# Kyo-suke-S/Depth_image_captioning_pub

Measured on AMD Instinct MI355X. Metric: images/sec (train, depth-soft, 224x224, seq-len 20), higher is better.
Workload: dtype f32; 1 GPU; depth-soft train step, synthetic RGB-D 224x224, batch 64/GPU, seq-len 20, V=10000, ResNet-152 (random init, batch-stat BN) + depth CNN + soft-attention LSTM; global_batch=64, batch_per_gpu=64, seq_len=20, vocab=10000, parallelism=dp1, resnet_conv_mode=f16x2, cross_step_resnet_overlap=True, resnet_forwards_in_flight=3, annotation_cells=49, ranks=1, collective=none (single rank)

## Files before the change

### depth_image_captioning_pub_amd/csrc/api.hip

```cpp
#include "dic.h"
#include "conv.h"
#include "nn_kernels.h"

#include <cstdio>

using namespace dic;

namespace dic { void resnet_fuse_bn_operand(int mask); void resnet_fuse_bn_halo(int on); void resnet_fuse_res_bn(int on); void depth_encoder_l1_sparse(int on); void bn_finalize_two_level_rows(int rows); void resnet_debug_fused_tail_bn(int on); void conv1_depth_debug_blocks(int n);
                void depth_encoder_f16x2(int on); }
#ifdef DIC_EXPERIMENTS
namespace dic { void decoder_debug_persistent(int on); void decoder_persist_debug_buffer(unsigned long long* p); void decoder_persist_debug_placement(int p);
                void resnet_debug_skip_bn_apply(int on); }
#endif

extern "C" {

int dic_version(void) { return DIC_ABI_VERSION; }
size_t dic_struct_bytes(int which) {
  switch (which) {
    case 0: return sizeof(dic_conv_bn_layer);
    case 1: return sizeof(dic_decoder_weights);
    case 2: return sizeof(dic_decoder_grads);
    case 3: return sizeof(dic_depth_encoder_weights);
    case 4: return sizeof(dic_depth_encoder_grads);
// ... 24 lines not shown
}

int dic_conv2d_fwd(const float* x, int B, int H, int W, int C, int in_nchw, const float* w_ohwi, const float* bias,
                   int CO, int KH, int KW, int stride, int pad, float* y_nhwc, float* bn_partial, int* mtiles_out,
                   int force_tile, float* tail_ws, void* stream) {
  ConvDesc d{B, H, W, C, CO, KH, KW, stride, pad, in_nchw};
  return conv_fwd(x, d, w_ohwi, bias, y_nhwc, bn_partial, mtiles_out, (hipStream_t)stream, force_tile, tail_ws);
}

int dic_debug_force_staged_gemm(int on) {
  if (gemm_bf3_force_tile(on) == 0) return 0;
  if (on >= 100 && on <= 104) { dic::resnet_fuse_bn_operand(on == 104 ? -1 : on - 100); return 0; }
  if (on == 98 || on == 99) { dic::resnet_fuse_res_bn(on - 98); return 0; }
  if (on == 108 || on == 109) { dic::resnet_fuse_bn_halo(on - 108); return 0; }
  if (on == 182 || on == 183) { dic::bn_finalize_two_level_rows(on == 182 ? 512 : 1024); return 0; }
  if (on == 180 || on == 181) { dic::depth_encoder_l1_sparse(on - 180); return 0; }
  if (on == 116 || on == 117) { dic::depth_encoder_f16x2(on - 116); return 0; }
#ifdef DIC_EXPERIMENTS
  if (on == 140 || on == 141) { dic::decoder_debug_persistent(on - 140); return 0; }
  if (on == 142 || on == 143) { dic::decoder_persist_debug_placement(on - 142); return 0; }
  if (on >= 130 && on <= 134) { dic::conv1_depth_debug_blocks(256 * (on - 130)); return 0; }
  if (on >= 150 && on <= 153) { dic::resnet_debug_fused_tail_bn(on - 150); return 0; }
  if (on >= 124 && on <= 127) { dic::resnet_debug_skip_bn_apply(on == 125 ? 3 : on == 126 ? 2 : on == 127 ? 1 : 0); return 0; }
  if (on >= 0 && on <= 13) { gemm_force_v1(on); return 0; }
#endif
  DIC_REQUIRE(false, "debug switch: unknown code %d", on);
  return 0;
}
#ifdef DIC_EXPERIMENTS
int dic_debug_decoder_stamps(unsigned long long* dev_buf) { dic::decoder_persist_debug_buffer(dev_buf); return 0; }
#endif
int dic_debug_conv1_wgrad(const float* x, int B, int H, int W, const float* dy, float* dw, float* dbias, float* ws, float* cs_ws,
                          void* stream) {
  ConvDesc d{B, H, W, 1, 128, 7, 7, 3, 0, 0};
  return conv1_depth_wgrad(x, d, dy, dw, dbias, ws, cs_ws, (hipStream_t)stream);
}
int dic_debug_conv1_fwd(const float* x, int B, int H, int W, const float* w, const float* bias, float* y, float* partial,
                        void* stream) {
  ConvDesc d{B, H, W, 1, 128, 7, 7, 3, 0, 0};
  int rows = 0;
  return conv1_depth_fwd(x, d, w, bias, y, partial, &rows, (hipStream_t)stream);
}
// ... 355 lines not shown
```

### depth_image_captioning_pub_amd/csrc/decoder.h

```cpp
#pragma once
#include "dic.h"
#include "gemm.h"
#include <vector>

namespace dic {

constexpr int kL = DIC_L, kD = DIC_D, kA = DIC_A, kE = DIC_E, kH = DIC_H;
constexpr int kG = 4 * kH;
constexpr int kXK = kE + kD + kH;
constexpr int kNCH = kD / 256;
constexpr int kLCH = 4;
constexpr int kLc = 49;
constexpr int kS_LSTM = 18;
constexpr int kS_DX = 4;

struct SetupBufs {
  float *F, *P, *mean, *Wcat, *WcatT, *bcat, *WhT, *WbT, *gemm_ws;
  size_t gemm_ws_floats;
};

struct DecoderWs : SetupBufs {
  float *WzT, *Xall, *Hall, *Call, *Gact, *Qall, *ctx, *gate, *Hdrop;
  float* slab_g;
  float *dHd, *dG, *slab_dx, *dctx, *dgpre, *dq, *dalp, *pbeta, *dqp, *dwf_acc, *dbf_acc, *dPacc, *carry_dc;
// ... 21 lines not shown
    constexpr int L_ = kL;              \
    STMT                                \
  } else {                              \
    constexpr int L_ = kLc;             \
    STMT                                \
  }

struct StepPlan { int T = 0, N = 0; std::vector<int> bs, off; };
int make_plan(const int* dec_len, int B, StepPlan* pl);

int launch_transpose(const float* in, float* out, int R, int Cc, hipStream_t st);
int gemm(int M, int N, int K, GemmOperand A, GemmOperand B, GemmEpilogue ep, hipStream_t st, int splitk = 1, float* ws = nullptr,
         int tile = 0, int raw_partials = 0);
int gemm_slabs(int M, int N, int K, GemmOperand A, GemmOperand B, float* slabs, int splitk, hipStream_t st);

struct InitState { float *h0, *c0; long long ld; bool WcatT; };
int decoder_setup(const dic_decoder_weights* w, const float* feat_rgb, const float* feat_depth, int B, int cells,
                  const SetupBufs& s, const InitState& o, hipStream_t st);

struct LstmCell {
  const float *slab, *bcat, *drop; float *Hall, *Call, *Gact, *Hdrop;
  int nslab, nb, packed_off;
};
int launch_lstm_fwd(const LstmCell& c, int t, int T, hipStream_t st);

struct FusedLstm : LstmCell { int nb_cur; };

struct AttnStepArgs {
  const float *F, *P, *Hall, *WhT, *b_h, *w_full, *b_full, *WbT, *b_beta;
  int t, T, mode; const float* gumbel_u; int B; float temp;
// ... 131 lines not shown
```

### depth_image_captioning_pub_amd/csrc/decoder_bwd.hip

```cpp
#include "decoder.h"
#include <algorithm>

namespace dic {

__global__ void __launch_bounds__(256) colsum_kernel(const float* __restrict__ X, long long ld, int M, int N,
                                                      float* __restrict__ out, int rs) {
  const int n = blockIdx.x * 256 + threadIdx.x;
  if (n >= N) return;
  float s = 0.f;
#pragma unroll 8
  for (int m = blockIdx.y; m < M; m += rs) s += X[(long long)m * ld + n];
  out[(long long)blockIdx.y * N + n] = s;
}

__global__ void __launch_bounds__(256) colsum_batch_kernel(const ColsumBatch b, int stage) {
  const ColsumJob job = b.j[blockIdx.z];
  const int n = blockIdx.x * 256 + threadIdx.x, y = blockIdx.y;
  if (n >= job.N) return;
  if (stage == 1) {
    if (y >= job.rs) return;
    float s = 0.f;
#pragma unroll 8
    for (int m = y; m < job.M; m += job.rs) s += job.X[(long long)m * job.ld + n];
    (job.rs > 1 ? job.part : job.out)[(long long)y * job.N + n] = s;
// ... 20 lines not shown
  if (maxrs > 1) hipLaunchKernelGGL(colsum_batch_kernel, dim3(ceil_div(maxn, 256), 1, njobs), dim3(256), 0, st, b, 2);
  DIC_LAUNCH_CHECK();
  return DIC_OK;
}

static int colsum(const float* X, long long ld, int M, int N, float* out, float* ws, hipStream_t st) {
  const int rs = std::min(64, std::max(1, M / 8));
  if (rs > 1) {
    hipLaunchKernelGGL(colsum_kernel, dim3(ceil_div(N, 256), rs), dim3(256), 0, st, X, ld, M, N, ws, rs);
    hipLaunchKernelGGL(colsum_kernel, dim3(ceil_div(N, 256), 1), dim3(256), 0, st, ws, (long long)N, rs, N, out, 1);
  } else {
    hipLaunchKernelGGL(colsum_kernel, dim3(ceil_div(N, 256), 1), dim3(256), 0, st, X, ld, M, N, out, 1);
  }
  DIC_LAUNCH_CHECK();
  return DIC_OK;
}

__global__ void __launch_bounds__(kH) lstm_bwd_kernel(const LstmBwdArgs la) { lstm_bwd_body(blockIdx.x, threadIdx.x, true, la); }

template <int L>
__global__ void __launch_bounds__(512, 4) attn_bwd_a_kernel(
    const float* __restrict__ F, const float* __restrict__ slab_dx, int nslab, int nb, int B, int t, int T,
    const float* __restrict__ ctx_all, const float* __restrict__ gate_all, const float* __restrict__ W_beta,
    const long long* __restrict__ cap, int cap_stride, int V, float* __restrict__ dctx_all,
    float* __restrict__ dgpre_all, float* __restrict__ dalp, float* __restrict__ pbeta, float* __restrict__ dembed) {
  __shared__ __align__(16) float dctx_s[256];
  __shared__ float dgp_s[256];
  __shared__ float pb_s[4][kH];
  __shared__ float da_s[256];
  const int chunk = blockIdx.x, b = blockIdx.y;
// ... 395 lines not shown
  DIC_REQUIRE(w != nullptr && workspace != nullptr, "decoder: null weights/workspace");
  DIC_REQUIRE(V > 0 && B > 0, "decoder: bad sizes");
  DIC_REQUIRE(g && dlogits_packed && alphas_in && captions, "decoder_bwd: null pointer");
  DIC_REQUIRE(mode == 0 || mode == 1, "decoder_bwd: only soft (0) and gumbel-softmax (1) attention are differentiable");
  StepPlan pl;
  DIC_TRY(make_plan(dec_lengths, B, &pl));
  const int T = pl.T, N = pl.N;
  DIC_REQUIRE(T <= 64, "decoder_bwd: at most 64 decode steps supported (got %d)", T);
  bool ov = false;
  DecoderWs ws = decoder_carve(workspace, workspace_bytes, B, T, V, N, &ov);
  DIC_REQUIRE(!ov, "decoder_bwd: workspace too small");
  const size_t BT = (size_t)B * T;

  int* d_len = ws.dlen;
  DIC_CHECK_HIP(hipMemcpyAsync(d_len, dec_lengths, sizeof(int) * B, hipMemcpyHostToDevice, st));
  DIC_CHECK_HIP(hipMemsetAsync(ws.dG, 0, (size_t)((char*)(ws.dq + BT * kA) - (char*)ws.dG), st));
  DIC_CHECK_HIP(hipMemsetAsync(g->embed, 0, sizeof(float) * (size_t)V * kE, st));
  float* cs = ws.colsum_ws;
  if (cells != kL) {
    alphas = ws.alpha_c;
    if (dalphas_in) {
      const long long n = (long long)B * T * kLc;
      hipLaunchKernelGGL(fold_dalphas_kernel, dim3((unsigned)((n + 255) / 256)), dim3(256), 0, st, dalphas_in, ws.dalpha_c, n);
      DIC_LAUNCH_CHECK();
      dalphas = ws.dalpha_c;
    }
  }

  DIC_TRY(gemm(N, kH, V, op_rowk(dlogits_packed, V), op_colk(w->out_w, kH), ep_store(ws.dHd, kH), st, 8, ws.gemm_ws));
  DIC_TRY(gemm(V, kH, N, op_colk(dlogits_packed, V), op_colk(ws.Hdrop, kH), ep_store(g->out_w, kH), st));
  DIC_TRY(colsum(dlogits_packed, V, N, V, g->out_b, cs, st));

  const float inv_temp = (mode == 1) ? 1.0f / temp : 1.0f;
  const bool fuse_b = (nlch == 1);
  auto lstm_args = [&](int t) {
    LstmBwdArgs a{};
    a.T = T; a.B = B; a.nlch = nlch; a.dHd = ws.dHd; a.drop = drop_mult; a.slab_dx = ws.slab_dx; a.nslab_dx = kS_DX;
    a.dqp = ws.dqp; a.pbeta = ws.pbeta; a.W_h = w->dec_att_w; a.Gact = ws.Gact; a.Call = ws.Call; a.carry_dc = ws.carry_dc;
    a.dG = ws.dG; a.dq_all = ws.dq; a.dinit = ws.dinit;
    if (t < 0) { a.t = -1; a.nb_next = pl.bs[0]; a.have_next = 1; a.final_pass = 1; a.packed_off = 0; a.nb_slab = pl.bs[0]; }
    else {
      a.t = t; a.have_next = (t + 1 < T); a.nb_next = a.have_next ? pl.bs[t + 1] : 0; a.final_pass = 0;
      a.packed_off = pl.off[t]; a.nb_slab = a.nb_next;
    }
    return a;
  };
// ... 119 lines not shown
```

### depth_image_captioning_pub_amd/csrc/gemm.h

```cpp
#pragma once
#include "common.h"

namespace dic {

__host__ __device__ __forceinline__ long long plane_offset(long long r, long long k, long long kblocks, int paired) {
  if (!paired) return r * kblocks * 32 + k;
  return (((r >> 1) * kblocks + (k >> 5)) << 6) + ((r & 1) << 5) + (k & 31);
}

enum : int { OPK_ROWK = 0, OPK_COLK = 1, OPK_IM2COL = 2, OPK_GATHER = 3, OPK_IM2COL_COLK = 4, OPK_GATHER_COLK = 5 };
enum : int { ACT_NONE = 0, ACT_RELU = 1, ACT_SIGMOID = 2, ACT_GELU = 3 };

struct ConvGeom {
  int H, W, C;
  int OH, OW;
  int KH, KW, stride, pad;
  int nchw;
};

struct GemmOperand {
  const float* p;
  long long ld;
  int kind;
  int vec;
// ... 16 lines not shown
};

struct GemmParams {
  int M, N, K;
  GemmOperand A, B;
  GemmEpilogue ep;
  int mtiles, ntiles;
  int splitk;
  int ktiles_per_split;
  float* ws;
  int tail_first_block, tail_first_tile, tail_split;
  float* tail_ws;
  int ablate;
  int raw_partials;
  int tail128_first, tail128_ntiles;
};

size_t gemm_splitk_ws_bytes(int M, int N, int splitk);
constexpr size_t kGemmTailWsBytes = (size_t)256 * 64 * 64 * sizeof(float);
int gemm_pick_tile(int M, int N);
int gemm_launch(GemmParams p, hipStream_t st, int force_tile = 0);
constexpr int kGemmGroupMax = 6;
int gemm_launch_group_colk(GemmParams* ps, int n, hipStream_t st);
GemmOperand op_rowk(const float* p, long long ld);
GemmOperand op_colk(const float* p, long long ld);
GemmOperand op_im2col(const float* x, const ConvGeom& g);
GemmOperand op_gather(const float* x, const ConvGeom& g);
GemmOperand op_im2col_colk(const float* x, const ConvGeom& g);
GemmOperand op_gather_colk(const float* x, const ConvGeom& g);
void gemm_force_v1(int on);
int gemm_bf3_set_persist_grid(int workgroups);
int gemm_bf3_force_tile(int code);
int gemm_launch_tail_fixup(const GemmParams& p, int tail_tiles, hipStream_t st);

struct BnFuseArgs {
// ... 25 lines not shown
```

### depth_image_captioning_pub_amd/csrc/gemm.hip

```cpp
#include "gemm.h"
#include "gemm_epilogue.h"
#include <algorithm>
#include <map>
#include <vector>

namespace dic {

constexpr int BK = 32;

template <int KIND>
struct KFast { static constexpr bool v = (KIND == OPK_ROWK || KIND == OPK_IM2COL || KIND == OPK_GATHER); };

template <int KIND, int BR>
struct Loader {
  static constexpr bool KFAST = KFast<KIND>::v;
  static constexpr int LD = KFAST ? BR + 1 : BR + 4;
  static constexpr int NV = BR / 32;
  static constexpr int I4 = BR / 4;
  static constexpr int KSTEP = 256 / I4;

  const float* p;
  long long ld;
  int R, K, vec;
  ConvGeom g;
// ... 530 lines not shown
    const float sc = bn.gamma[c] * invstd;
    bn.scale[c] = sc;
    bn.shift[c] = bn.beta[c] - (float)mean * sc;
    bn.mean[c] = (float)mean;
    bn.invstd[c] = invstd;
    const bool finite = fabs(a) <= 1.7e308 && fabs(b) <= 1.7e308;
    if (!finite) f16x2_raise(bn.status, 8u);
    if (bn.running_mean && finite) {
      const double unb = bn.count > 1.0 ? var * bn.count / (bn.count - 1.0) : var;
      bn.running_mean[c] = fmaf(1.f - bn.momentum, bn.running_mean[c], __fmul_rn(bn.momentum, (float)mean));
      bn.running_var[c] = fmaf(1.f - bn.momentum, bn.running_var[c], __fmul_rn(bn.momentum, (float)unb));
    }
  }
}

template <int BM, int BN, int AK, int BKIND, int ABL = 0>
__device__ __forceinline__ void gemm_tile_body(const GemmParams& p, const int bid, const int nblk) {
  using LA = Loader<AK, BM>;
  using LB = Loader<BKIND, BN>;
  constexpr int LDA = LA::LD, LDB = LB::LD;
  constexpr int WM = BM / 2, WN = BN / 2, TM = WM / 32, TN = WN / 32;
  __shared__ __align__(16) float As[2][BK * LDA];
  __shared__ __align__(16) float Bs[2][BK * LDB];

  const int tid = threadIdx.x, lane = tid & 63, wave = tid >> 6;
  const int wm = wave >> 1, wn = wave & 1;
  const int lb = xcd_remap(bid, nblk);
  const int tiles = p.mtiles * p.ntiles;
  const int z = lb / tiles, t = lb - z * tiles;
  const int tm = t / p.ntiles, tn = t - tm * p.ntiles;

  LA la;
// ... 16 lines not shown
  }

  const int nk = (p.K + BK - 1) / BK;
  const int kt0 = z * p.ktiles_per_split;
  const int kt1 = min(nk, kt0 + p.ktiles_per_split);

  f32x16 acc[TM][TN];
#pragma unroll
  for (int i = 0; i < TM; ++i)
#pragma unroll
    for (int j = 0; j < TN; ++j)
#pragma unroll
      for (int r = 0; r < 16; ++r) acc[i][j][r] = 0.f;

  float4 ra[LA::NV], rb[LB::NV];
  const int nkt = kt1 - kt0;
  if (nkt > 0) {
    la.load(kt0 * BK, ra);
    lbld.load(kt0 * BK, rb);
    la.store(As[0], ra);
    lbld.store(Bs[0], rb);
  }
  if (nkt > 1) {
    la.load((kt0 + 1) * BK, ra);
    lbld.load((kt0 + 1) * BK, rb);
  }
  __syncthreads();

  const int arow = wm * WM + (lane & 31);
  const int brow = wn * WN + (lane & 31);
  const int khalf = lane >> 5;
  for (int it = 0; it < nkt; ++it) {
    const int cur = it & 1;
    if (ABL == 0 || ABL == 3) {
    if (it + 1 < nkt) {
      la.store(As[cur ^ 1], ra);
      lbld.store(Bs[cur ^ 1], rb);
    }
    if (it + 2 < nkt && ABL == 0) {
      la.load((kt0 + it + 2) * BK, ra);
      lbld.load((kt0 + it + 2) * BK, rb);
    }
    }
    const float* Ac = As[cur] + khalf * LDA + arow;
    const float* Bc = Bs[cur] + khalf * LDB + brow;
    float af[TM][BK / 2], bf[TN][BK / 2];
#pragma unroll
    for (int kk = 0; kk < BK / 2; ++kk) {
#pragma unroll
      for (int i = 0; i < TM; ++i) af[i][kk] = (ABL == 2) ? (float)(it + kk + i) : Ac[kk * 2 * LDA + i * 32];
#pragma unroll
      for (int j = 0; j < TN; ++j) bf[j][kk] = (ABL == 2) ? (float)(it - kk + j) : Bc[kk * 2 * LDB + j * 32];
    }
    __builtin_amdgcn_sched_barrier(0);
#pragma unroll
    for (int kk = 0; kk < BK / 2; ++kk)
#pragma unroll
      for (int i = 0; i < TM; ++i)
#pragma unroll
        for (int j = 0; j < TN; ++j)
          acc[i][j] = __builtin_amdgcn_mfma_f32_32x32x2f32(af[i][kk], bf[j][kk], acc[i][j], 0, 0, 0);
    __syncthreads();
  }

  gemm_epilogue<BM, BN>(p, acc, tm, tn, z, As[0]);
}

template <int BM, int BN, int AK, int BKIND, int ABL = 0>
__global__ void __launch_bounds__(256) gemm_kernel(const GemmParams p) {
  gemm_tile_body<BM, BN, AK, BKIND, ABL>(p, blockIdx.x, gridDim.x);
}

struct GemmGroup {
  int n;
  int first[kGemmGroupMax + 1];
  GemmParams p[kGemmGroupMax];
};
static_assert(sizeof(GemmGroup) <= 4096, "GemmGroup travels as a kernel argument");
template <int BM, int BN, int AK, int BKIND>
__global__ void __launch_bounds__(256) gemm_group_kernel(const GemmGroup g) {
  int i = 0;
#pragma unroll
  for (int j = 1; j < kGemmGroupMax; ++j)
    if (j < g.n && (int)blockIdx.x >= g.first[j]) i = j;
  gemm_tile_body<BM, BN, AK, BKIND>(g.p[i], (int)blockIdx.x - g.first[i], g.first[i + 1] - g.first[i]);
}

__device__ __forceinline__ void splitk_reduce_body(const GemmParams& p, const int bid, const int nblk) {
  const long long total = (long long)p.M * p.N;
  const float alpha = ep_alpha(p.ep);
  for (long long e = (long long)bid * 256 + threadIdx.x; e < total; e += (long long)nblk * 256) {
    float s = 0.f;
    for (int z = 0; z < p.splitk; ++z) s += p.ws[(long long)z * total + e];
    const int m = (int)(e / p.N), n = (int)(e - (long long)m * p.N);
    finalize_store(p.ep, m, n, s, alpha);
  }
}
__global__ void __launch_bounds__(256) splitk_reduce_kernel(const GemmParams p) { splitk_reduce_body(p, blockIdx.x, gridDim.x); }
__global__ void __launch_bounds__(256) splitk_reduce_group_kernel(const GemmGroup g) {
  int i = 0;
#pragma unroll
  for (int j = 1; j < kGemmGroupMax; ++j)
    if (j < g.n && (int)blockIdx.x >= g.first[j]) i = j;
  splitk_reduce_body(g.p[i], (int)blockIdx.x - g.first[i], g.first[i + 1] - g.first[i]);
}

struct ProfRec { hipEvent_t e0, e1; double flops; int key; double bytes; };
static bool g_prof_on = false;
static bool g_force_v1 = false;
static int g_dma_stages = 2;
static bool g_tail_split_on = true;
// ... 96 lines not shown
  GemmEpilogue e{};
  e.C = C; e.ldc = ldc; e.bias = bias; e.act = act; e.alpha = 1.0f;
  return e;
}

size_t gemm_splitk_ws_bytes(int M, int N, int splitk) {
  return splitk > 1 ? (size_t)splitk * M * N * sizeof(float) : 0;
}

int gemm_pick_tile(int M, int N) {
  const long long t128 = (long long)ceil_div(M, 128) * ceil_div(N, 128);
  if (N >= 128 && M >= 128 && t128 >= 4096) return 128;
  return 64;
}

template <int BM, int BN>
static int launch_tile(const GemmParams& p, hipStream_t st) {
  const dim3 grid(p.mtiles * p.ntiles * p.splitk), block(256);
  const int a = p.A.kind, b = p.B.kind;
#define DIC_GEMM_CASE(AK_, BK_)                                                     \
  if (a == AK_ && b == BK_) {                                                       \
    hipLaunchKernelGGL((gemm_kernel<BM, BN, AK_, BK_>), grid, block, 0, st, p);     \
    return DIC_OK;                                                                  \
  }
  if (a == OPK_ROWK && b == OPK_ROWK && p.ablate > 0) {
    if (p.ablate == 1) hipLaunchKernelGGL((gemm_kernel<BM, BN, OPK_ROWK, OPK_ROWK, 1>), grid, block, 0, st, p);
    else if (p.ablate == 2) hipLaunchKernelGGL((gemm_kernel<BM, BN, OPK_ROWK, OPK_ROWK, 2>), grid, block, 0, st, p);
    else hipLaunchKernelGGL((gemm_kernel<BM, BN, OPK_ROWK, OPK_ROWK, 3>), grid, block, 0, st, p);
    return DIC_OK;
  }
// ... 42 lines not shown
  if (p.A.kind == OPK_IM2COL) DIC_REQUIRE(p.A.g.C % 32 == 0, "im2col loader needs C %% 32 == 0 (C=%d)", p.A.g.C);
  const bool taps_ok = p.A.kind != OPK_IM2COL || p.A.g.KH * p.A.g.KW <= 32;
  if (p.B.kind == OPK_IM2COL_COLK) DIC_REQUIRE(p.B.g.C % 4 == 0, "im2col_colk loader needs C %% 4 == 0");
  const int tile = force_tile ? force_tile : gemm_pick_tile(p.M, p.N);
  p.mtiles = ceil_div(p.M, tile);
  p.ntiles = ceil_div(p.N, tile);
  const int nk = ceil_div(p.K, BK);
  if (p.splitk < 1) p.splitk = 1;
  if (p.splitk > nk) p.splitk = nk;
  p.ktiles_per_split = ceil_div(nk, p.splitk);
  p.splitk = ceil_div(nk, p.ktiles_per_split);
  if (p.splitk > 1) {
    DIC_REQUIRE(p.ws != nullptr, "gemm: split-K needs a workspace");
    DIC_REQUIRE(p.ep.stats == nullptr, "gemm: BN statistics epilogue cannot be combined with split-K");
  }
  if (p.ep.alpha == 0.0f) p.ep.alpha = 1.0f;
  const bool dma_ok = (p.B.kind == OPK_ROWK && p.B.vec && (p.K % 4 == 0) && p.ablate == 0 && !g_force_v1 && taps_ok &&
                       (p.A.kind == OPK_IM2COL || (p.A.kind == OPK_ROWK && p.A.vec)));
  int total_blocks = p.mtiles * p.ntiles * p.splitk;
  p.tail_first_block = total_blocks; p.tail_first_tile = 0; p.tail_split = 1;
  int tail_tiles = 0;
  if (dma_ok && tile == 64 && p.splitk == 1 && p.tail_ws != nullptr && g_tail_split_on) {
    const int T = p.mtiles * p.ntiles, r = T % 256;
    int s = r > 0 ? 256 / r : 0;
    s = std::min(s, std::min(nk / 2, kTailMaxSplit));
    if (r > 0 && r <= 128 && s >= 2 && T < 7 * 256) {
      tail_tiles = r;
      p.tail_first_tile = T - r;
      p.tail_first_block = T - r;
      p.tail_split = s;
// ... 12 lines not shown
  int rc = DIC_OK;
  if (dma_ok) {
    const dim3 grid(total_blocks), block(256);
    if (tile == 128) {
      if (p.A.kind == OPK_IM2COL) hipLaunchKernelGGL((gemm_dma_kernel<128, 128, OPK_IM2COL, 2>), grid, block, 0, st, p);
      else hipLaunchKernelGGL((gemm_dma_kernel<128, 128, OPK_ROWK, 2>), grid, block, 0, st, p);
    } else if (p.raw_partials && p.A.kind == OPK_ROWK && p.mtiles == 1 && p.ktiles_per_split <= 8) {
      hipLaunchKernelGGL((gemm_dma_kernel<64, 64, OPK_ROWK, 4>), grid, block, 0, st, p);
    } else if (g_dma_stages == 2) {
      if (p.A.kind == OPK_IM2COL) hipLaunchKernelGGL((gemm_dma_kernel<64, 64, OPK_IM2COL, 2>), grid, block, 0, st, p);
      else hipLaunchKernelGGL((gemm_dma_kernel<64, 64, OPK_ROWK, 2>), grid, block, 0, st, p);
    } else {
      if (p.A.kind == OPK_IM2COL) hipLaunchKernelGGL((gemm_dma_kernel<64, 64, OPK_IM2COL, 3>), grid, block, 0, st, p);
      else hipLaunchKernelGGL((gemm_dma_kernel<64, 64, OPK_ROWK, 3>), grid, block, 0, st, p);
    }
  } else {
    rc = (tile == 128) ? launch_tile<128, 128>(p, st) : launch_tile<64, 64>(p, st);
  }
  if (rc != 0) return rc;
  DIC_LAUNCH_CHECK();
  if (tail_tiles > 0 && !g_tail_skip_fix) {
    const dim3 g(tail_tiles), b(1024);
  if (p.tail_split <= 2) hipLaunchKernelGGL(tail_fixup_kernel<2>, g, b, 0, st, p);
  else if (p.tail_split <= 4) hipLaunchKernelGGL(tail_fixup_kernel<4>, g, b, 0, st, p);
  else if (p.tail_split <= 8) hipLaunchKernelGGL(tail_fixup_kernel<8>, g, b, 0, st, p);
  else hipLaunchKernelGGL(tail_fixup_kernel<16>, g, b, 0, st, p);
    DIC_LAUNCH_CHECK();
  }
  if (g_prof_on) {
    (void)hipEventRecord(rec.e1, st);
// ... 64 lines not shown
```

### depth_image_captioning_pub_amd/csrc/nic_train.hip

```cpp
#include "nic.h"
#include <algorithm>

namespace dic {

struct NicTape {
  float *G0, *C0, *H0, *H0p, *G1, *C1, *H1p, *Hdrop;
};

__global__ void __launch_bounds__(kNicThreads) nic_lstm2_seq_fwd(const float* __restrict__ Gx0, const float* __restrict__ Whh0p,
                                                                  const float* __restrict__ Wih1p, const float* __restrict__ Whh1p,
                                                                  const float* __restrict__ b1, const int* __restrict__ dlen,
                                                                  const int* __restrict__ off, const float* __restrict__ drop,
                                                                  int B, int T, NicTape tp) {
  __shared__ __align__(16) float h0_s[kNicR][kH];
  __shared__ __align__(16) float h1_s[kNicR][kH];
  __shared__ __align__(16) float g_s[kNicR][kG];
  const int tid = threadIdx.x, b0 = blockIdx.x * kNicR;
  const int rc = tid >> 7, u = tid & (kH - 1), bc = b0 + rc;
  const __amdgpu_buffer_rsrc_t Whh0 = nic_rsrc(Whh0p, kG * kH), Wih1 = nic_rsrc(Wih1p, kG * kH), Whh1 = nic_rsrc(Whh1p, kG * kH);
  int len[kNicR];
#pragma unroll
  for (int r = 0; r < kNicR; ++r) len[r] = b0 + r < B ? dlen[b0 + r] : 0;
  const int mylen = bc < B ? dlen[bc] : 0;
  const int steps = len[0];
// ... 77 lines not shown
                                                                const NicPackPlan pl, long long* __restrict__ out) {
  const int t = blockIdx.x, o = pl.off[t], nb = pl.bs[t];
  for (int b = threadIdx.x; b < nb; b += 256) out[o + b] = cap[(long long)b * cap_stride + t0 + t];
}

namespace {

constexpr int kNicSplitDH = 8;

struct NicWs {
  NicStepWs fw;
  float *Wih1B, *Whh1B, *Whh0B;
  float *X, *Gx0, *dG1, *dHd, *dX, *gemm_ws, *cs_ws;
  NicTape tp;
  int *dlen, *off, *tok;
  size_t bytes;
};

NicWs nic_carve(void* p, size_t bytes, int B, int T, int V, int N, bool* overflow) {
  Carver c(p, bytes);
  NicWs w{};
  const size_t n = (size_t)N;
  for (float** m : {&w.fw.Whh0F, &w.fw.Wih1F, &w.fw.Whh1F, &w.Wih1B, &w.Whh1B, &w.Whh0B}) *m = c.take<float>((size_t)kG * kH);
  w.fw.bsum0 = c.take<float>(kG);
  w.fw.bsum1 = c.take<float>(kG);
  w.dlen = c.take<int>((size_t)B);
  w.off = c.take<int>((size_t)T + 1);
  w.tok = c.take<int>(n);
  w.X = c.take<float>(n * kNicE);
  w.Gx0 = c.take<float>(n * kG);
  w.tp.G0 = c.take<float>(n * kG);
  w.tp.G1 = c.take<float>(n * kG);
  for (float** m : {&w.tp.C0, &w.tp.H0, &w.tp.H0p, &w.tp.C1, &w.tp.H1p, &w.tp.Hdrop, &w.dHd}) *m = c.take<float>(n * kH);
  w.dG1 = c.take<float>(n * kG);
  w.dX = c.take<float>(n * kNicE);
  w.gemm_ws = c.take<float>((size_t)kNicSplitDH * n * kH);
  w.cs_ws = c.take<float>((size_t)256 * std::max(V, kG));
  w.bytes = c.off;
  if (overflow) *overflow = c.overflow;
  return w;
}

int nic_check_lengths(const char* who, const int* lengths, int B, int cap_stride, StepPlan* pl) {
  DIC_REQUIRE(lengths != nullptr, "%s: null pointer (lengths)", who);
  for (int b = 0; b < B; ++b) {
    DIC_REQUIRE(lengths[b] >= 1, "%s: lengths[%d]=%d is < 1", who, b, lengths[b]);
    DIC_REQUIRE(lengths[b] <= cap_stride, "%s: lengths[%d]=%d is > cap_stride=%d", who, b, lengths[b], cap_stride);
    DIC_REQUIRE(b == 0 || lengths[b] <= lengths[b - 1], "%s: lengths are not descending (lengths[%d]=%d > lengths[%d]=%d)", who, b,
                lengths[b], b - 1, lengths[b - 1]);
  }
  return make_plan(lengths, B, pl);
// ... 41 lines not shown
                const float* drop_mult, const float* dlogits_packed, const dic_nic_grads* g, float* d_features, void* workspace,
                size_t workspace_bytes, void* stream) {
  hipStream_t st = (hipStream_t)stream;
  DIC_REQUIRE(B > 0, "dic_nic_bwd: bad batch size B=%d", B);
  DIC_REQUIRE(V > 0, "dic_nic_bwd: bad vocabulary size V=%d", V);
  DIC_REQUIRE(w && captions && dlogits_packed && g && d_features && workspace, "dic_nic_bwd: null pointer");
  DIC_REQUIRE(g->embed && g->w_ih_l0 && g->w_hh_l0 && g->b_ih_l0 && g->b_hh_l0 && g->w_ih_l1 && g->w_hh_l1 && g->b_ih_l1 &&
                  g->b_hh_l1 && g->out_w && g->out_b, "dic_nic_bwd: null pointer (gradient table)");
  StepPlan pl;
  if (int rc = nic_check_lengths("dic_nic_bwd", lengths, B, cap_stride, &pl)) return rc;
  const int T = pl.T, N = pl.N;
  bool ov = false;
  NicWs ws = nic_carve(workspace, workspace_bytes, B, T, V, N, &ov);
  if (ov) return workspace_too_small("dic_nic_bwd", workspace_bytes, ws.bytes);
  float *dG0 = ws.Gx0, *dG1 = ws.dG1;
  DIC_TRY(gemm(N, kH, V, op_rowk(dlogits_packed, V), op_colk(w->out_w, kH), ep_store(ws.dHd, kH), st, kNicSplitDH, ws.gemm_ws));
  DIC_TRY(gemm(V, kH, N, op_colk(dlogits_packed, V), op_colk(ws.tp.Hdrop, kH), ep_store(g->out_w, kH), st));
  DIC_TRY(colsum_rows(dlogits_packed, V, N, V, g->out_b, ws.cs_ws, st));
  DIC_TRY(nic_bwd_setup(w, ws.Wih1B, ws.Whh1B, ws.Whh0B, st));
  hipLaunchKernelGGL(nic_lstm2_seq_bwd, dim3(ceil_div(B, kNicR)), dim3(kNicThreads), 0, st, ws.dHd, drop_mult, ws.Wih1B,
                     ws.Whh1B, ws.Whh0B, ws.dlen, ws.off, B, T, ws.tp, dG0, dG1);
  DIC_LAUNCH_CHECK();
  DIC_TRY(nic_grad_tail(w, g, N, dG0, dG1, ws.tp.H0, ws.tp.H0p, ws.tp.H1p, ws.X, ws.dX, ws.cs_ws, st));
  DIC_CHECK_HIP(hipMemcpyAsync(d_features, ws.dX, sizeof(float) * B * kNicE, hipMemcpyDeviceToDevice, st));
  return nic_embed_grad("dic_nic_bwd", "n_packed", ws.dX, ws.tok, N, N > B, V, g->embed, st);
}

int dic_nic_pack_targets(const int64_t* captions, int cap_stride, const int* lengths, int B, int64_t* targets, void* stream) {
  hipStream_t st = (hipStream_t)stream;
  DIC_REQUIRE(B > 0, "dic_nic_pack_targets: bad batch size B=%d", B);
  DIC_REQUIRE(captions && targets, "dic_nic_pack_targets: null pointer");
  StepPlan pl;
  if (int rc = nic_check_lengths("dic_nic_pack_targets", lengths, B, cap_stride, &pl)) return rc;
// ... 13 lines not shown
```

### depth_image_captioning_pub_amd/csrc/train_ops.hip

```cpp
#include "dic.h"
#include "common.h"
#include <algorithm>
#include <cmath>
#include <vector>

namespace dic {

template <bool SMOOTH>
__global__ void __launch_bounds__(256) ce_fwd_bwd_kernel(const float* logits,
                                                          const long long* __restrict__ targets, int V, float gscale,
                                                          float eps, float* __restrict__ loss_rows,
                                                          float* __restrict__ nll_rows, float* dlogits) {
  __shared__ float red[8];
  __shared__ double redx[4];
  const int row = blockIdx.x, tid = threadIdx.x, lane = tid & 63, w = tid >> 6;
  const float* x = logits + (long long)row * V;
  float m = -INFINITY;
  for (int v = tid; v < V; v += 256) m = fmaxf(m, x[v]);
  m = wave_max(m);
  if (lane == 0) red[w] = m;
  __syncthreads();
  m = fmaxf(fmaxf(red[0], red[1]), fmaxf(red[2], red[3]));
  float s = 0.f;
  double sx = 0.0;
  if constexpr (SMOOTH) {
    for (int v = tid; v < V; v += 256) {
      const float xv = x[v];
      s += expf(xv - m);
      sx += (double)xv;
    }
#pragma unroll
    for (int o = 32; o > 0; o >>= 1) sx += __shfl_xor(sx, o, 64);
    if (lane == 0) redx[w] = sx;
  } else {
    for (int v = tid; v < V; v += 256) s += expf(x[v] - m);
  }
  s = wave_sum(s);
  if (lane == 0) red[4 + w] = s;
  __syncthreads();
  s = red[4] + red[5] + red[6] + red[7];
  const float lse = m + logf(s);
  long long tg = targets[row];
  const bool bad_target = tg < 0 || tg >= V;
  tg = tg < 0 ? 0 : (tg >= V ? V - 1 : tg);
  if constexpr (SMOOTH) {
    if (tid == 0) {
      const float xt = x[tg];
      const float nll_row = lse - xt;
      const float mean = (float)((redx[0] + redx[1] + redx[2] + redx[3]) / (double)V);
      const float smooth_row = eps == 0.f ? nll_row : (lse - (1.f - eps) * xt) - eps * mean;
      loss_rows[row] = bad_target ? __builtin_nanf("") : smooth_row;
      nll_rows[row] = bad_target ? __builtin_nanf("") : nll_row;
    }
  } else {
    if (tid == 0) loss_rows[row] = bad_target ? __builtin_nanf("") : lse - x[tg];
  }
  __threadfence_block();
  __syncthreads();
  float* dx = dlogits + (long long)row * V;
  if constexpr (SMOOTH) {
    const float on = 1.f - eps, u = eps / (float)V;
    for (int v = tid; v < V; v += 256) {
      const float p = expf(x[v] - lse);
      dx[v] = ((p - (v == tg ? on : 0.f)) - u) * gscale;
    }
  } else {
    for (int v = tid; v < V; v += 256) {
      const float p = expf(x[v] - lse);
      dx[v] = (p - (v == tg ? 1.f : 0.f)) * gscale;
    }
  }
}

__global__ void __launch_bounds__(256) alpha_reg_kernel(const float* __restrict__ alphas, int T, float coef,
                                                         float* __restrict__ reg_rows, float* __restrict__ dalphas) {
  __shared__ float red[4];
  const int b = blockIdx.x, tid = threadIdx.x, lane = tid & 63, w = tid >> 6;
  float r = 0.f;
  if (tid < DIC_L) {
    float s = 0.f;
    for (int t = 0; t < T; ++t) s += alphas[((long long)b * T + t) * DIC_L + tid];
    r = 1.f - s;
    const float g = -2.f * r * coef;
    for (int t = 0; t < T; ++t) dalphas[((long long)b * T + t) * DIC_L + tid] = g;
  }
  const float p = wave_sum(r * r);
  if (lane == 0) red[w] = p;
// ... 94 lines not shown
      out[i] = (u >= p) ? scale : 0.f;
    }
  }
}

}

using namespace dic;

extern "C" {

static int caption_loss_launch(const float* logits, const int64_t* targets, int n_packed, int V, const float* alphas, int B,
                               int Tmax, float lam, float eps, float ce_grad_scale, float reg_grad_scale, float* loss, float* nll,
                               float* dlogits, float* dalphas, float* loss_rows, float* nll_rows, float* reg_rows, hipStream_t st) {
  const float gscale = ce_grad_scale / (float)n_packed;
  if (nll_rows)
    hipLaunchKernelGGL(ce_fwd_bwd_kernel<true>, dim3(n_packed), dim3(256), 0, st, logits, (const long long*)targets, V, gscale, eps,
                       loss_rows, nll_rows, dlogits);
  else
    hipLaunchKernelGGL(ce_fwd_bwd_kernel<false>, dim3(n_packed), dim3(256), 0, st, logits, (const long long*)targets, V, gscale, 0.f,
                       loss_rows, (float*)nullptr, dlogits);
  DIC_LAUNCH_CHECK();
  float reg_scale = 0.f;
  if (alphas) {
    reg_scale = lam / ((float)B * (float)DIC_L);
    hipLaunchKernelGGL(alpha_reg_kernel, dim3(B), dim3(256), 0, st, alphas, Tmax, reg_scale * reg_grad_scale, reg_rows,
                       dalphas);
    DIC_LAUNCH_CHECK();
  }
  hipLaunchKernelGGL(loss_finish_kernel, dim3(1), dim3(256), 0, st, loss_rows, n_packed,
                     alphas ? reg_rows : (const float*)nullptr, B, reg_scale, loss);
  DIC_LAUNCH_CHECK();
  if (nll) {
    hipLaunchKernelGGL(loss_finish_kernel, dim3(1), dim3(256), 0, st, nll_rows, n_packed, (const float*)nullptr, B, 0.f, nll);
    DIC_LAUNCH_CHECK();
  }
// ... 92 lines not shown
```

### include/dic.h

```cpp
#ifndef DIC_H_
#define DIC_H_
#include <stddef.h>
#include <stdint.h>

#ifdef __cplusplus
extern "C" {
#endif

#define DIC_L 196
#define DIC_D 2048
#define DIC_A 128
#define DIC_E 128
#define DIC_H 128

#define DIC_ABI_VERSION 200
int dic_version(void);
const char* dic_last_error(void);
size_t dic_struct_bytes(int which);

int dic_gemm_f32(int M, int N, int K, const float* A, long long lda, int a_colk, const float* B, long long ldb,
                 int b_colk, float* C, long long ldc, const float* bias, int act, int accumulate, int splitk,
                 float* workspace, size_t workspace_bytes, int force_tile, void* stream);

int dic_conv2d_fwd(const float* x, int B, int H, int W, int C, int in_nchw, const float* w_ohwi, const float* bias,
// ... 346 lines not shown
int dic_add_act(const float* a, const float* b, long long n, long long period, int act, float* out, void* stream);
int dic_pointwise_dot(const float* x, long long rows, int C, const float* w, const float* bias, int relu, float* out,
                      void* stream);

int dic_normalize_images(const float* in, float* out, int B, int C, int H, int W, const float* mean3, const float* std3,
                         void* stream);
int dic_resize_bilinear(const float* in, int planes, int H, int W, int resize_short, int crop, float mul, float add,
                        float* out, void* stream);
int dic_depth_standardize(float* depth, int B, long long hw, void* stream);
int dic_bn_ema_update(float* running, const float* delta, long long n, float momentum, void* stream);
int dic_bn_ema_update_guarded(float* running, const float* delta, long long n, float momentum, const uint32_t* skip_if_raised,
                              void* stream);
int dic_gather_rows(const float* table, const int64_t* idx, int n, long long row_floats, float* out, void* stream);

int dic_debug_force_staged_gemm(int on);
int dic_debug_bn_finalize(const float* partial, int mtiles, long long count, int C, const float* gamma, const float* beta,
                          float* running_mean, float* running_var, float* scale, float* shift, float* mean, float* invstd, double* red,
                          size_t red_doubles, uint32_t* status, void* stream);
int dic_debug_bn_finalize_eval(int C, const float* gamma, const float* beta, const float* running_mean, const float* running_var,
                               float* scale, float* shift, float* mean, float* invstd, void* stream);
int dic_debug_bn_apply(const float* x, const float* residual, const uint16_t* const residual_planes[3], float* y, uint16_t* const planes[3],
                       long long rows, int C, const float* scale, const float* shift, const float* mean, const float* invstd, int relu,
                       const float* res_scale, const float* res_shift, const float* res_mean, const float* res_invstd, uint32_t* status,
                       void* stream);
int dic_debug_bn_relu_maxpool(const float* x, int B, int H, int W, int C, const float* scale, const float* shift, const float* mean,
                              const float* invstd, int relu, int k, int s, int p, float* y, unsigned char* idx, uint16_t* const planes[3],
                              uint32_t* status, float* xsel, void* stream);
int dic_debug_adaptive_avgpool(const float* x, int B, int H, int W, int C, const float* scale, const float* shift, const float* mean,
                               const float* invstd, int relu, int out, float* y, void* stream);
int dic_debug_adaptive_avgpool_bwd(const float* dy, int B, int H, int W, int C, int out, float* dx, void* stream);
// ... 49 lines not shown
```

Before: 7547 images/s.

## Split-K vocab head backward with fused bias colsum; keep CE logits row in registers

The vocab-projection backward now picks split-K counts adaptively so both the dHd and dW GEMMs fill the GPU, and it borrows the decoder gradient block as split-K workspace before that block is zeroed. The output-bias column sum is fused into the dW GEMM's K-major A loader, which drops a separate pass over dlogits. The cross-entropy kernel caches each logits row in registers (up to 10240 entries) instead of reading it from global memory three times. The costs are more register pressure in the CE kernel, extra split-K reduce traffic, and reordering the memset so the workspace can be reused.

```diff
diff --git a/depth_image_captioning_pub_amd/csrc/api.hip b/depth_image_captioning_pub_amd/csrc/api.hip
--- a/depth_image_captioning_pub_amd/csrc/api.hip
+++ b/depth_image_captioning_pub_amd/csrc/api.hip
@@ -7,7 +7,8 @@
 using namespace dic;
 
 namespace dic { void resnet_fuse_bn_operand(int mask); void resnet_fuse_bn_halo(int on); void resnet_fuse_res_bn(int on); void depth_encoder_l1_sparse(int on); void bn_finalize_two_level_rows(int rows); void resnet_debug_fused_tail_bn(int on); void conv1_depth_debug_blocks(int n);
-                void depth_encoder_f16x2(int on); }
+                void depth_encoder_f16x2(int on); void caption_loss_row_in_registers(int on); void vocab_head_bwd_policy(int on);
+                size_t vocab_head_bwd_ws_floats(int N, int V); size_t vocab_head_scratch_bytes(int B, int T); }
 #ifdef DIC_EXPERIMENTS
 namespace dic { void decoder_debug_persistent(int on); void decoder_persist_debug_buffer(unsigned long long* p); void decoder_persist_debug_placement(int p);
                 void resnet_debug_skip_bn_apply(int on); }
@@ -62,6 +63,8 @@
   if (on == 98 || on == 99) { dic::resnet_fuse_res_bn(on - 98); return 0; }
   if (on == 108 || on == 109) { dic::resnet_fuse_bn_halo(on - 108); return 0; }
   if (on == 182 || on == 183) { dic::bn_finalize_two_level_rows(on == 182 ? 512 : 1024); return 0; }
+  if (on == 188 || on == 189) { dic::caption_loss_row_in_registers(on - 188); return 0; }
+  if (on == 186 || on == 187) { dic::vocab_head_bwd_policy(on - 186); return 0; }
   if (on == 180 || on == 181) { dic::depth_encoder_l1_sparse(on - 180); return 0; }
   if (on == 116 || on == 117) { dic::depth_encoder_f16x2(on - 116); return 0; }
 #ifdef DIC_EXPERIMENTS
@@ -74,6 +77,19 @@
 #endif
   DIC_REQUIRE(false, "debug switch: unknown code %d", on);
   return 0;
+}
+int dic_debug_gemm_splitk(int M, int N, int K, size_t ws_floats, int* out) {
+  DIC_REQUIRE(M > 0 && N > 0 && K > 0 && out, "dic_debug_gemm_splitk: bad arguments (M=%d, N=%d, K=%d)", M, N, K);
+  const int s = gemm_pick_splitk(M, N, K, ws_floats), nk = (K + 31) / 32, per = (nk + s - 1) / s;
+  out[0] = s; out[1] = per; out[2] = nk - (s - 1) * per; out[3] = ((M + 63) / 64) * ((N + 63) / 64) * s;
+  return DIC_OK;
+}
+int dic_debug_vocab_head_ws_floats(int B, int Tmax, int n_packed, int V, size_t* out) {
+  DIC_REQUIRE(B > 0 && Tmax > 0 && n_packed > 0 && V > 0 && out, "dic_debug_vocab_head_ws_floats: bad arguments (B=%d, Tmax=%d, n_packed=%d, V=%d)", B,
+              Tmax, n_packed, V);
+  out[0] = dic::vocab_head_scratch_bytes(B, Tmax) / sizeof(float);
+  out[1] = dic::vocab_head_bwd_ws_floats(n_packed, V);
+  return DIC_OK;
 }
 #ifdef DIC_EXPERIMENTS
 int dic_debug_decoder_stamps(unsigned long long* dev_buf) { dic::decoder_persist_debug_buffer(dev_buf); return 0; }
diff --git a/depth_image_captioning_pub_amd/csrc/decoder.h b/depth_image_captioning_pub_amd/csrc/decoder.h
--- a/depth_image_captioning_pub_amd/csrc/decoder.h
+++ b/depth_image_captioning_pub_amd/csrc/decoder.h
@@ -59,6 +59,14 @@
          int tile = 0, int raw_partials = 0);
 int gemm_slabs(int M, int N, int K, GemmOperand A, GemmOperand B, float* slabs, int splitk, hipStream_t st);
 
+size_t vocab_head_scratch_bytes(int B, int T);
+constexpr int kVocabHeadMaxSlices = 64;
+size_t vocab_head_bwd_ws_floats(int N, int V);
+void vocab_head_bwd_policy(int on);
+bool vocab_head_bwd_sliced();
+int vocab_head_bwd(const float* dlogits, int N, int V, const float* out_w, const float* Hdrop, float* dHd, float* g_out_w,
+                   float* g_out_b, float* gemm_ws, size_t gemm_ws_floats, float* colsum_ws, hipStream_t st);
+
 struct InitState { float *h0, *c0; long long ld; bool WcatT; };
 int decoder_setup(const dic_decoder_weights* w, const float* feat_rgb, const float* feat_depth, int B, int cells,
                   const SetupBufs& s, const InitState& o, hipStream_t st);
diff --git a/depth_image_captioning_pub_amd/csrc/decoder_bwd.hip b/depth_image_captioning_pub_amd/csrc/decoder_bwd.hip
--- a/depth_image_captioning_pub_amd/csrc/decoder_bwd.hip
+++ b/depth_image_captioning_pub_amd/csrc/decoder_bwd.hip
@@ -58,6 +58,39 @@
   }
   DIC_LAUNCH_CHECK();
   return DIC_OK;
+}
+
+static bool g_vocab_head_sliced = true;
+void vocab_head_bwd_policy(int on) { g_vocab_head_sliced = on != 0; }
+bool vocab_head_bwd_sliced() { return g_vocab_head_sliced; }
+size_t vocab_head_scratch_bytes(int B, int T) {
+  const size_t BT = (size_t)B * T;
+  auto taken = [](size_t floats) { return (floats * sizeof(float) + 255) & ~size_t(255); };
+  return taken(BT * kG) + 2 * taken(BT * kD) + BT * kA * sizeof(float);
+}
+
+static size_t vocab_head_dw_cap(int V) { return (size_t)kVocabHeadMaxSlices * V * kH; }
+
+size_t vocab_head_bwd_ws_floats(int N, int V) {
+  const size_t dh = (size_t)gemm_pick_splitk(N, kH, V, (size_t)-1) * N * kH;
+  const size_t dw = (size_t)gemm_pick_splitk(V, kH, N, vocab_head_dw_cap(V)) * V * kH;
+  return std::max(std::max(dh, dw), (size_t)8 * N * kH);
+}
+
+int vocab_head_bwd(const float* dlogits, int N, int V, const float* out_w, const float* Hdrop, float* dHd, float* g_out_w,
+                   float* g_out_b, float* gemm_ws, size_t gemm_ws_floats, float* colsum_ws, hipStream_t st) {
+  if (!g_vocab_head_sliced) {
+    DIC_TRY(gemm(N, kH, V, op_rowk(dlogits, V), op_colk(out_w, kH), ep_store(dHd, kH), st, 8, gemm_ws));
+    DIC_TRY(gemm(V, kH, N, op_colk(dlogits, V), op_colk(Hdrop, kH), ep_store(g_out_w, kH), st));
+    return colsum(dlogits, V, N, V, g_out_b, colsum_ws, st);
+  }
+  DIC_TRY(gemm(N, kH, V, op_rowk(dlogits, V), op_colk(out_w, kH), ep_store(dHd, kH), st,
+               gemm_pick_splitk(N, kH, V, gemm_ws_floats), gemm_ws));
+  GemmParams p{};
+  p.M = V; p.N = kH; p.K = N; p.A = op_colk(dlogits, V); p.B = op_colk(Hdrop, kH); p.ep = ep_store(g_out_w, kH);
+  p.splitk = gemm_pick_splitk(V, kH, N, std::min(gemm_ws_floats, vocab_head_dw_cap(V)));
+  p.ws = gemm_ws; p.colsum_out = g_out_b; p.colsum_ws = colsum_ws;
+  return gemm_launch(p, st, 64);
 }
 
 __global__ void __launch_bounds__(kH) lstm_bwd_kernel(const LstmBwdArgs la) { lstm_bwd_body(blockIdx.x, threadIdx.x, true, la); }
@@ -483,7 +516,6 @@
 
   int* d_len = ws.dlen;
   DIC_CHECK_HIP(hipMemcpyAsync(d_len, dec_lengths, sizeof(int) * B, hipMemcpyHostToDevice, st));
-  DIC_CHECK_HIP(hipMemsetAsync(ws.dG, 0, (size_t)((char*)(ws.dq + BT * kA) - (char*)ws.dG), st));
   DIC_CHECK_HIP(hipMemsetAsync(g->embed, 0, sizeof(float) * (size_t)V * kE, st));
   float* cs = ws.colsum_ws;
   if (cells != kL) {
@@ -496,9 +528,9 @@
     }
   }
 
-  DIC_TRY(gemm(N, kH, V, op_rowk(dlogits_packed, V), op_colk(w->out_w, kH), ep_store(ws.dHd, kH), st, 8, ws.gemm_ws));
-  DIC_TRY(gemm(V, kH, N, op_colk(dlogits_packed, V), op_colk(ws.Hdrop, kH), ep_store(g->out_w, kH), st));
-  DIC_TRY(colsum(dlogits_packed, V, N, V, g->out_b, cs, st));
+  const size_t grad_block = (size_t)((char*)(ws.dq + BT * kA) - (char*)ws.dG);
+  DIC_TRY(vocab_head_bwd(dlogits_packed, N, V, w->out_w, ws.Hdrop, ws.dHd, g->out_w, g->out_b, ws.dG, grad_block / sizeof(float), cs, st));
+  DIC_CHECK_HIP(hipMemsetAsync(ws.dG, 0, grad_block, st));
 
   const float inv_temp = (mode == 1) ? 1.0f / temp : 1.0f;
   const bool fuse_b = (nlch == 1);
diff --git a/depth_image_captioning_pub_amd/csrc/gemm.h b/depth_image_captioning_pub_amd/csrc/gemm.h
--- a/depth_image_captioning_pub_amd/csrc/gemm.h
+++ b/depth_image_captioning_pub_amd/csrc/gemm.h
@@ -54,11 +54,15 @@
   int ablate;
   int raw_partials;
   int tail128_first, tail128_ntiles;
+  float* colsum_out;
+  float* colsum_ws;
 };
 
 size_t gemm_splitk_ws_bytes(int M, int N, int splitk);
 constexpr size_t kGemmTailWsBytes = (size_t)256 * 64 * 64 * sizeof(float);
 int gemm_pick_tile(int M, int N);
+constexpr int kGemmSplitTarget = 1024, kGemmSplitMinTiles = 4;
+int gemm_pick_splitk(int M, int N, int K, size_t ws_floats);
 int gemm_launch(GemmParams p, hipStream_t st, int force_tile = 0);
 constexpr int kGemmGroupMax = 6;
 int gemm_launch_group_colk(GemmParams* ps, int n, hipStream_t st);
diff --git a/depth_image_captioning_pub_amd/csrc/gemm.hip b/depth_image_captioning_pub_amd/csrc/gemm.hip
--- a/depth_image_captioning_pub_amd/csrc/gemm.hip
+++ b/depth_image_captioning_pub_amd/csrc/gemm.hip
@@ -568,8 +568,9 @@
   }
 }
 
-template <int BM, int BN, int AK, int BKIND, int ABL = 0>
+template <int BM, int BN, int AK, int BKIND, int ABL = 0, bool CS = false>
 __device__ __forceinline__ void gemm_tile_body(const GemmParams& p, const int bid, const int nblk) {
+  static_assert(!CS || (AK == OPK_COLK && BM == 64), "the column sum rides on the K-major loader of a 64-row tile");
   using LA = Loader<AK, BM>;
   using LB = Loader<BKIND, BN>;
   constexpr int LDA = LA::LD, LDB = LB::LD;
@@ -616,12 +617,19 @@
       for (int r = 0; r < 16; ++r) acc[i][j][r] = 0.f;
 
   float4 ra[LA::NV], rb[LB::NV];
+  float4 csum = make_float4(0.f, 0.f, 0.f, 0.f);
+  const bool cs_on = CS && tn == 0;
+  auto cs_add = [&]() {
+#pragma unroll
+    for (int r = 0; r < LA::NV; ++r) { csum.x += ra[r].x; csum.y += ra[r].y; csum.z += ra[r].z; csum.w += ra[r].w; }
+  };
   const int nkt = kt1 - kt0;
   if (nkt > 0) {
     la.load(kt0 * BK, ra);
     lbld.load(kt0 * BK, rb);
     la.store(As[0], ra);
     lbld.store(Bs[0], rb);
+    if (cs_on) cs_add();
   }
   if (nkt > 1) {
     la.load((kt0 + 1) * BK, ra);
@@ -638,6 +646,7 @@
     if (it + 1 < nkt) {
       la.store(As[cur ^ 1], ra);
       lbld.store(Bs[cur ^ 1], rb);
+      if (cs_on) cs_add();
     }
     if (it + 2 < nkt && ABL == 0) {
       la.load((kt0 + it + 2) * BK, ra);
@@ -665,12 +674,30 @@
     __syncthreads();
   }
 
+  if constexpr (CS) {
+    if (cs_on) {
+      float* sc = As[0];
+      *reinterpret_cast<float4*>(sc + la.kk0 * BM + la.i4 * 4) = csum;
+      __syncthreads();
+      if (tid < BM) {
+        float s = 0.f;
+#pragma unroll
+        for (int q = 0; q < LA::KSTEP; ++q) s += sc[q * BM + tid];
+        const int m = tm * BM + tid;
+        if (m < p.M) (p.splitk > 1 ? p.colsum_ws[(long long)z * p.M + m] : p.colsum_out[m]) = s;
+      }
+      __syncthreads();
+    }
+  }
   gemm_epilogue<BM, BN>(p, acc, tm, tn, z, As[0]);
 }
 
 template <int BM, int BN, int AK, int BKIND, int ABL = 0>
 __global__ void __launch_bounds__(256) gemm_kernel(const GemmParams p) {
   gemm_tile_body<BM, BN, AK, BKIND, ABL>(p, blockIdx.x, gridDim.x);
+}
+__global__ void __launch_bounds__(256) gemm_colk_colsum_kernel(const GemmParams p) {
+  gemm_tile_body<64, 64, OPK_COLK, OPK_COLK, 0, true>(p, blockIdx.x, gridDim.x);
 }
 
 struct GemmGroup {
@@ -697,6 +724,12 @@
     const int m = (int)(e / p.N), n = (int)(e - (long long)m * p.N);
     finalize_store(p.ep, m, n, s, alpha);
   }
+  if (p.colsum_out)
+    for (int e = bid * 256 + threadIdx.x; e < p.M; e += nblk * 256) {
+      float s = 0.f;
+      for (int z = 0; z < p.splitk; ++z) s += p.colsum_ws[(long long)z * p.M + e];
+      p.colsum_out[e] = s;
+    }
 }
 __global__ void __launch_bounds__(256) splitk_reduce_kernel(const GemmParams p) { splitk_reduce_body(p, blockIdx.x, gridDim.x); }
 __global__ void __launch_bounds__(256) splitk_reduce_group_kernel(const GemmGroup g) {
@@ -823,6 +856,21 @@
   return 64;
 }
 
+int gemm_pick_splitk(int M, int N, int K, size_t ws_floats) {
+  if (M <= 0 || N <= 0 || K <= 0) return 1;
+  const long long tiles = (long long)ceil_div(M, 64) * ceil_div(N, 64);
+  const int nk = ceil_div(K, BK);
+  const long long want = (kGemmSplitTarget + tiles - 1) / tiles;
+  int per = (int)std::max<long long>(nk / want, std::min(nk, kGemmSplitMinTiles));
+  int s = ceil_div(nk, per);
+  const size_t cap = std::max<size_t>(ws_floats / ((size_t)M * N), 1);
+  if ((size_t)s > cap) {
+    per = ceil_div(nk, (int)cap);
+    s = ceil_div(nk, per);
+  }
+  return s;
+}
+
 template <int BM, int BN>
 static int launch_tile(const GemmParams& p, hipStream_t st) {
   const dim3 grid(p.mtiles * p.ntiles * p.splitk), block(256);
@@ -895,6 +943,9 @@
     DIC_REQUIRE(p.ws != nullptr, "gemm: split-K needs a workspace");
     DIC_REQUIRE(p.ep.stats == nullptr, "gemm: BN statistics epilogue cannot be combined with split-K");
   }
+  if (p.colsum_out)
+    DIC_REQUIRE(p.A.kind == OPK_COLK && p.B.kind == OPK_COLK && tile == 64 && !p.raw_partials && p.ablate == 0 &&
+                (p.splitk == 1 || p.colsum_ws != nullptr), "gemm: the fused column sum takes K-major operands, 64x64 tiles and its own split-K slab");
   if (p.ep.alpha == 0.0f) p.ep.alpha = 1.0f;
   const bool dma_ok = (p.B.kind == OPK_ROWK && p.B.vec && (p.K % 4 == 0) && p.ablate == 0 && !g_force_v1 && taps_ok &&
                        (p.A.kind == OPK_IM2COL || (p.A.kind == OPK_ROWK && p.A.vec)));
@@ -937,6 +988,8 @@
       if (p.A.kind == OPK_IM2COL) hipLaunchKernelGGL((gemm_dma_kernel<64, 64, OPK_IM2COL, 3>), grid, block, 0, st, p);
       else hipLaunchKernelGGL((gemm_dma_kernel<64, 64, OPK_ROWK, 3>), grid, block, 0, st, p);
     }
+  } else if (p.colsum_out) {
+    hipLaunchKernelGGL(gemm_colk_colsum_kernel, dim3(total_blocks), dim3(256), 0, st, p);
   } else {
     rc = (tile == 128) ? launch_tile<128, 128>(p, st) : launch_tile<64, 64>(p, st);
   }
diff --git a/depth_image_captioning_pub_amd/csrc/nic_train.hip b/depth_image_captioning_pub_amd/csrc/nic_train.hip
--- a/depth_image_captioning_pub_amd/csrc/nic_train.hip
+++ b/depth_image_captioning_pub_amd/csrc/nic_train.hip
@@ -115,6 +115,7 @@
   float *X, *Gx0, *dG1, *dHd, *dX, *gemm_ws, *cs_ws;
   NicTape tp;
   int *dlen, *off, *tok;
+  size_t gemm_ws_floats;
   size_t bytes;
 };
 
@@ -135,7 +136,8 @@
   for (float** m : {&w.tp.C0, &w.tp.H0, &w.tp.H0p, &w.tp.C1, &w.tp.H1p, &w.tp.Hdrop, &w.dHd}) *m = c.take<float>(n * kH);
   w.dG1 = c.take<float>(n * kG);
   w.dX = c.take<float>(n * kNicE);
-  w.gemm_ws = c.take<float>((size_t)kNicSplitDH * n * kH);
+  w.gemm_ws_floats = vocab_head_bwd_ws_floats(N, V);
+  w.gemm_ws = c.take<float>(w.gemm_ws_floats);
   w.cs_ws = c.take<float>((size_t)256 * std::max(V, kG));
   w.bytes = c.off;
   if (overflow) *overflow = c.overflow;
@@ -207,9 +209,14 @@
   NicWs ws = nic_carve(workspace, workspace_bytes, B, T, V, N, &ov);
   if (ov) return workspace_too_small("dic_nic_bwd", workspace_bytes, ws.bytes);
   float *dG0 = ws.Gx0, *dG1 = ws.dG1;
-  DIC_TRY(gemm(N, kH, V, op_rowk(dlogits_packed, V), op_colk(w->out_w, kH), ep_store(ws.dHd, kH), st, kNicSplitDH, ws.gemm_ws));
-  DIC_TRY(gemm(V, kH, N, op_colk(dlogits_packed, V), op_colk(ws.tp.Hdrop, kH), ep_store(g->out_w, kH), st));
-  DIC_TRY(colsum_rows(dlogits_packed, V, N, V, g->out_b, ws.cs_ws, st));
+  if (vocab_head_bwd_sliced()) {
+    DIC_TRY(vocab_head_bwd(dlogits_packed, N, V, w->out_w, ws.tp.Hdrop, ws.dHd, g->out_w, g->out_b, ws.gemm_ws, ws.gemm_ws_floats,
+                           ws.cs_ws, st));
+  } else {
+    DIC_TRY(gemm(N, kH, V, op_rowk(dlogits_packed, V), op_colk(w->out_w, kH), ep_store(ws.dHd, kH), st, kNicSplitDH, ws.gemm_ws));
+    DIC_TRY(gemm(V, kH, N, op_colk(dlogits_packed, V), op_colk(ws.tp.Hdrop, kH), ep_store(g->out_w, kH), st));
+    DIC_TRY(colsum_rows(dlogits_packed, V, N, V, g->out_b, ws.cs_ws, st));
+  }
   DIC_TRY(nic_bwd_setup(w, ws.Wih1B, ws.Whh1B, ws.Whh0B, st));
   hipLaunchKernelGGL(nic_lstm2_seq_bwd, dim3(ceil_div(B, kNicR)), dim3(kNicThreads), 0, st, ws.dHd, drop_mult, ws.Wih1B,
                      ws.Whh1B, ws.Whh0B, ws.dlen, ws.off, B, T, ws.tp, dG0, dG1);
diff --git a/depth_image_captioning_pub_amd/csrc/train_ops.hip b/depth_image_captioning_pub_amd/csrc/train_ops.hip
--- a/depth_image_captioning_pub_amd/csrc/train_ops.hip
+++ b/depth_image_captioning_pub_amd/csrc/train_ops.hip
@@ -6,7 +6,8 @@
 
 namespace dic {
 
-template <bool SMOOTH>
+constexpr int kCeRowRegs = 40;
+template <bool SMOOTH, bool REG>
 __global__ void __launch_bounds__(256) ce_fwd_bwd_kernel(const float* logits,
                                                           const long long* __restrict__ targets, int V, float gscale,
                                                           float eps, float* __restrict__ loss_rows,
@@ -15,8 +16,22 @@
   __shared__ double redx[4];
   const int row = blockIdx.x, tid = threadIdx.x, lane = tid & 63, w = tid >> 6;
   const float* x = logits + (long long)row * V;
+  float xr[REG ? kCeRowRegs : 1];
+  if constexpr (REG) {
+#pragma unroll
+    for (int j = 0; j < kCeRowRegs; ++j) xr[j] = tid + 256 * j < V ? x[tid + 256 * j] : 0.f;
+  }
+  auto each = [&](auto&& f) {
+    if constexpr (REG) {
+#pragma unroll
+      for (int j = 0; j < kCeRowRegs; ++j)
+        if (tid + 256 * j < V) f(tid + 256 * j, xr[j]);
+    } else {
+      for (int v = tid; v < V; v += 256) f(v, x[v]);
+    }
+  };
   float m = -INFINITY;
-  for (int v = tid; v < V; v += 256) m = fmaxf(m, x[v]);
+  each([&](int, float xv) { m = fmaxf(m, xv); });
   m = wave_max(m);
   if (lane == 0) red[w] = m;
   __syncthreads();
@@ -24,16 +39,15 @@
   float s = 0.f;
   double sx = 0.0;
   if constexpr (SMOOTH) {
-    for (int v = tid; v < V; v += 256) {
-      const float xv = x[v];
+    each([&](int, float xv) {
       s += expf(xv - m);
       sx += (double)xv;
-    }
+    });
 #pragma unroll
     for (int o = 32; o > 0; o >>= 1) sx += __shfl_xor(sx, o, 64);
     if (lane == 0) redx[w] = sx;
   } else {
-    for (int v = tid; v < V; v += 256) s += expf(x[v] - m);
+    each([&](int, float xv) { s += expf(xv - m); });
   }
   s = wave_sum(s);
   if (lane == 0) red[4 + w] = s;
@@ -60,17 +74,19 @@
   float* dx = dlogits + (long long)row * V;
   if constexpr (SMOOTH) {
     const float on = 1.f - eps, u = eps / (float)V;
-    for (int v = tid; v < V; v += 256) {
-      const float p = expf(x[v] - lse);
+    each([&](int v, float xv) {
+      const float p = expf(xv - lse);
       dx[v] = ((p - (v == tg ? on : 0.f)) - u) * gscale;
-    }
+    });
   } else {
-    for (int v = tid; v < V; v += 256) {
-      const float p = expf(x[v] - lse);
+    each([&](int v, float xv) {
+      const float p = expf(xv - lse);
       dx[v] = (p - (v == tg ? 1.f : 0.f)) * gscale;
-    }
-  }
-}
+    });
+  }
+}
+static bool g_ce_row_in_registers = true;
+void caption_loss_row_in_registers(int on) { g_ce_row_in_registers = on != 0; }
 
 __global__ void __launch_bounds__(256) alpha_reg_kernel(const float* __restrict__ alphas, int T, float coef,
                                                          float* __restrict__ reg_rows, float* __restrict__ dalphas) {
@@ -195,12 +211,16 @@
                                int Tmax, float lam, float eps, float ce_grad_scale, float reg_grad_scale, float* loss, float* nll,
                                float* dlogits, float* dalphas, float* loss_rows, float* nll_rows, float* reg_rows, hipStream_t st) {
   const float gscale = ce_grad_scale / (float)n_packed;
-  if (nll_rows)
-    hipLaunchKernelGGL(ce_fwd_bwd_kernel<true>, dim3(n_packed), dim3(256), 0, st, logits, (const long long*)targets, V, gscale, eps,
-                       loss_rows, nll_rows, dlogits);
-  else
-    hipLaunchKernelGGL(ce_fwd_bwd_kernel<false>, dim3(n_packed), dim3(256), 0, st, logits, (const long long*)targets, V, gscale, 0.f,
-                       loss_rows, (float*)nullptr, dlogits);
+  const bool reg = g_ce_row_in_registers && V <= 256 * kCeRowRegs;
+  const dim3 grid(n_packed), block(256);
+  const long long* tg = (const long long*)targets;
+  if (nll_rows) {
+    if (reg) hipLaunchKernelGGL((ce_fwd_bwd_kernel<true, true>), grid, block, 0, st, logits, tg, V, gscale, eps, loss_rows, nll_rows, dlogits);
+    else hipLaunchKernelGGL((ce_fwd_bwd_kernel<true, false>), grid, block, 0, st, logits, tg, V, gscale, eps, loss_rows, nll_rows, dlogits);
+  } else {
+    if (reg) hipLaunchKernelGGL((ce_fwd_bwd_kernel<false, true>), grid, block, 0, st, logits, tg, V, gscale, 0.f, loss_rows, (float*)nullptr, dlogits);
+    else hipLaunchKernelGGL((ce_fwd_bwd_kernel<false, false>), grid, block, 0, st, logits, tg, V, gscale, 0.f, loss_rows, (float*)nullptr, dlogits);
+  }
   DIC_LAUNCH_CHECK();
   float reg_scale = 0.f;
   if (alphas) {
diff --git a/include/dic.h b/include/dic.h
--- a/include/dic.h
+++ b/include/dic.h
@@ -384,6 +384,8 @@
 int dic_gather_rows(const float* table, const int64_t* idx, int n, long long row_floats, float* out, void* stream);
 
 int dic_debug_force_staged_gemm(int on);
+int dic_debug_gemm_splitk(int M, int N, int K, size_t ws_floats, int* out);
+int dic_debug_vocab_head_ws_floats(int B, int Tmax, int n_packed, int V, size_t* out);
 int dic_debug_bn_finalize(const float* partial, int mtiles, long long count, int C, const float* gamma, const float* beta,
                           float* running_mean, float* running_var, float* scale, float* shift, float* mean, float* invstd, double* red,
                           size_t red_doubles, uint32_t* status, void* stream);
```

Result: slower. 7453 images/s (-1.2%).
